# puzzlepaint/surfelmeshing

Hardware: AMD Instinct MI355X
Metric: RGB-D frames/s integrated @640x480, 5M live surfels; achieved HBM GB/s (higher is better)
Workload: dtype f32; 1 GPU; C2: synthetic room stream 640x480, raw depth + colour frames resident in HBM, full preprocessing + Integrate per frame, 4912850 live surfels (6250000 slots), steady-state re-traversal; max_surfel_count=6250000, streams=1, parallelism=1 independent stream per GPU

## Files before the change

include/smx.h:

```cpp
#ifndef SMX_H_
#define SMX_H_

#include <stddef.h>
#include <stdint.h>

#ifdef __cplusplus
extern "C" {
#endif

typedef enum {
  SMX_OK = 0,
  SMX_ERR_INVALID_ARGUMENT = -1,
  SMX_ERR_HIP = -2,
  SMX_ERR_NO_DEVICE = -3,
  SMX_ERR_UNSUPPORTED = -4
} smx_status;

typedef void* smx_stream;
typedef struct smx_buffer_s* smx_buffer;
typedef struct smx_recon_s* smx_recon;
typedef struct smx_nn_s* smx_nn;

typedef struct {
  void* address;
// ... 150 lines not shown
int smx_recon_debug_internal_stream(smx_recon r, smx_stream* out);
int smx_recon_debug_stamp_ring(smx_recon r, uint64_t* out, int32_t capacity_words, int32_t* wall_clock_khz);
int smx_recon_set_timing_enabled(smx_recon r, int32_t enabled);
int smx_recon_kernel_slot_count(void);
const char* smx_recon_kernel_slot_name(int32_t slot);
int smx_recon_get_kernel_timings(smx_recon r, float* out_ms, int32_t capacity);
int smx_recon_profile_begin(smx_recon r, int32_t slot, int32_t max_frames);
int smx_recon_profile_end(smx_recon r, float* avg_ms, int32_t* frames);
int smx_recon_counts(smx_recon r, smx_stream s, uint32_t* surfel_count, uint32_t* surfels_size);

typedef struct {
  uint32_t surfels_size, merge_count;
  uint32_t n_visible;
  uint32_t n_new, n_merged, n_recent, n_edges;
  uint32_t n_integrated, n_replaced, n_conflict_hits;
  uint32_t capacity_clamped;
  uint32_t n_window_edges;
  uint32_t n_contributors;
  uint32_t n_segments_skipped;
  uint32_t regularizer_saturated;
  uint32_t n_pairs;
  uint32_t n_overflow_pairs;
  uint32_t max_tile_pairs;
} smx_recon_stats;
int smx_recon_get_stats(smx_recon r, smx_stream s, smx_recon_stats* out);
int smx_recon_set_stats_enabled(smx_recon r, int32_t enabled);

int smx_recon_debug_download_surfels(smx_recon r, smx_stream s, float* rows, uint32_t count);
int smx_recon_debug_upload_surfels(smx_recon r, smx_stream s, const float* rows, uint32_t count,
                                   uint32_t merge_count);
enum {
  SMX_SCRATCH_SUPPORTING = 0,
  SMX_SCRATCH_SUPPORT_COUNTS = 1,
  SMX_SCRATCH_DEPTH_SUMS = 2,
  SMX_SCRATCH_CONFLICTING = 3,
  SMX_SCRATCH_FIRST_DEPTH = 4,
  SMX_SCRATCH_NEW_FLAGS = 5,
  SMX_SCRATCH_NEW_INDICES = 6
};
int smx_recon_debug_download_scratch(smx_recon r, smx_stream s, int32_t which, void* dst);
int smx_recon_debug_count_skipped_segments(smx_recon r, smx_stream s, uint32_t* out);
int smx_recon_set_scan_mode(smx_recon r, int32_t mode);
int smx_recon_debug_set_skip(smx_recon r, int32_t mask);
int smx_recon_set_overlap(smx_recon r, int32_t enabled);
int smx_recon_integrate_hooks(smx_recon r, smx_event inputs_consumed, smx_event chain_after);
int smx_recon_integrate_inputs_ready(smx_recon r, smx_event inputs_ready);
// ... 520 lines not shown
```

surfelmeshing_amd/_lib.py:

```python
import ctypes as C
import os

os.environ.setdefault("GPU_MAX_HW_QUEUES", "8")
_HERE = os.path.dirname(os.path.abspath(__file__))
SO_PATH = os.environ.get("SMX_LIB_PATH") or os.path.join(_HERE, "libsmx.so")


class SmxError(RuntimeError):
    pass


class BufferDesc(C.Structure):
    _fields_ = [("address", C.c_void_p), ("height", C.c_int32), ("width", C.c_int32), ("pitch", C.c_size_t)]


class IntegrateParams(C.Structure):
    _fields_ = [("sensor_noise_factor", C.c_float),
                ("max_surfel_confidence", C.c_float),
                ("regularizer_weight", C.c_float),
                ("regularization_frame_window_size", C.c_int32),
                ("do_blending", C.c_int32),
                ("measurement_blending_radius", C.c_int32),
                ("regularization_iterations_per_integration_iteration", C.c_int32),
                ("radius_factor_for_regularization_neighbors", C.c_float),
# ... 325 lines not shown
    _fields_ = [(n, C.c_uint32) for n in ("n_in", "n_out_of_range", "n_not_live", "n_clipped", "n_degenerate", "n_culled",
                                          "n_drawn", "n_large", "n_covered_pixels")]


class SurfelBuffersCPU(C.Structure):
    _fields_ = [("frame_index", C.c_uint32), ("surfel_count", C.c_size_t),
                ("surfel_x_buffer", C.c_void_p), ("surfel_y_buffer", C.c_void_p), ("surfel_z_buffer", C.c_void_p),
                ("surfel_radius_squared_buffer", C.c_void_p),
                ("surfel_normal_x_buffer", C.c_void_p), ("surfel_normal_y_buffer", C.c_void_p),
                ("surfel_normal_z_buffer", C.c_void_p), ("surfel_last_update_stamp_buffer", C.c_void_p)]


class SurfelDeltaCPU(C.Structure):
    _fields_ = [("capacity", C.c_uint32), ("count", C.c_uint32), ("frame_index", C.c_uint32), ("surfel_count", C.c_uint32),
                ("surfel_index", C.c_void_p), ("x", C.c_void_p), ("y", C.c_void_p), ("z", C.c_void_p),
                ("radius_squared", C.c_void_p), ("normal_x", C.c_void_p), ("normal_y", C.c_void_p),
                ("normal_z", C.c_void_p), ("last_update_stamp", C.c_void_p)]


class ReconStats(C.Structure):
    _fields_ = [(n, C.c_uint32) for n in
                ("surfels_size", "merge_count", "n_visible", "n_new", "n_merged", "n_recent", "n_edges",
                 "n_integrated", "n_replaced", "n_conflict_hits", "capacity_clamped", "n_window_edges", "n_contributors",
                 "n_segments_skipped", "regularizer_saturated", "n_pairs", "n_overflow_pairs", "max_tile_pairs")]


class NNStats(C.Structure):
    _fields_ = [("n_points", C.c_uint32), ("n_indexed", C.c_uint32), ("n_bricks", C.c_uint32), ("cell_size", C.c_float),
                ("dim", C.c_int32 * 3), ("key_bits", C.c_int32), ("tiles", C.c_uint64), ("staged_candidates", C.c_uint64),
                ("distance_tests", C.c_uint64), ("results", C.c_uint64)]


EXPORTS = [
    "smx_last_error", "smx_runtime_advice", "smx_host_is_page_locked", "smx_device_count", "smx_set_device", "smx_device_name",
    "smx_stream_create", "smx_stream_create_with_priority", "smx_stream_create_with_cu_mask", "smx_recon_set_internal_cu_mask", "smx_recon_set_handover_mode", "smx_recon_get_handover_mode", "smx_host_alloc", "smx_host_free", "smx_stream_destroy", "smx_stream_synchronize", "smx_debug_marker", "smx_debug_handover_probe",
    "smx_debug_live_allocations", "smx_debug_fail_allocation",
    "smx_event_create", "smx_event_create_timed", "smx_event_elapsed_ms", "smx_event_destroy", "smx_event_record", "smx_stream_wait_event",
    "smx_buffer_create", "smx_buffer_destroy", "smx_buffer_get_desc", "smx_buffer_upload", "smx_buffer_upload_by_kernel", "smx_buffer_download",
    "smx_buffer_upload_part", "smx_buffer_download_part", "smx_buffer_clear", "smx_buffer_set_to",
    "smx_bilateral_filtering_and_depth_cutoff", "smx_outlier_depth_map_fusion", "smx_bilateral_outlier_fusion", "smx_erode_depth_map",
    "smx_copy_without_border", "smx_median_filter_and_densify_depth_map", "smx_downscale_using_median_while_excluding", "smx_color_image_pyramid", "smx_compute_normals_and_drop_bad_pixels",
    "smx_compute_point_radii_and_remove_isolated_pixels", "smx_erode_normals_radii", "smx_erode_normals_radii_signal",
    "smx_recon_create", "smx_recon_destroy", "smx_recon_integrate", "smx_recon_regularize",
    "smx_recon_transfer_all_to_cpu", "smx_recon_set_delta_tracking", "smx_recon_transfer_changed_to_cpu", "smx_recon_export_vertices", "smx_recon_get_timings", "smx_recon_get_timings_nowait", "smx_recon_debug_stamp_ring", "smx_recon_debug_internal_stream",
    "smx_recon_build_neighbor_index", "smx_recon_neighbor_candidates", "smx_recon_check_triangles",
    "smx_mesh_params_default", "smx_recon_triangulate", "smx_recon_debug_mesh_timings",
    "smx_recon_triangulate_update", "smx_recon_triangulate_reset", "smx_recon_debug_mesh_update_timings", "smx_recon_deform_by_creation_frame",
# ... 62 lines not shown
```

surfelmeshing_amd/csrc/smx_recon.hip:

```cpp
#include <math.h>
#include <cmath>
#include <stdlib.h>
#include <string.h>

#include <algorithm>
#include <atomic>
#include <vector>

#include "smx_recon_state.hpp"
#include "smx_mesh.hpp"
#include <hip/hip_ext.h>

using namespace smx;

namespace {

struct FrameCtx {
  Mat34 L;
  Mat34 G;
  float fx, fy, cx, cy;
  Unproj up;
  float inv_depth_scaling;
  float sensor_noise_factor;
  float cos_normal_compat;
// ... 165 lines not shown

__device__ __forceinline__ void keep(uint32_t v) { asm volatile("" :: "v"(v)); }
__device__ __forceinline__ void keep(int v) { asm volatile("" :: "v"(v)); }
__device__ __forceinline__ void keep(float v) { asm volatile("" :: "v"(v)); }
__device__ __forceinline__ void keep(const float2& v) { keep(v.x); keep(v.y); }
__device__ __forceinline__ void keep(const float4& v) { keep(v.x); keep(v.y); keep(v.z); keep(v.w); }
__device__ __forceinline__ void keep(const uint2& v) { keep(v.x); keep(v.y); }
__device__ __forceinline__ void keep(const uint4& v) { keep(v.x); keep(v.y); keep(v.z); keep(v.w); }

__device__ __forceinline__ void SMX_SET_WAVE_PRIO() { __builtin_amdgcn_s_setprio(1); }
typedef uint32_t v4u_t __attribute__((ext_vector_type(4)));
__device__ __forceinline__ void out_store16(void* p, const v4u_t& w) { *reinterpret_cast<v4u_t*>(p) = w; }
__device__ __forceinline__ void out_store16(void* p, const uint4& v) { const v4u_t w = {v.x, v.y, v.z, v.w}; out_store16(p, w); }
__device__ __forceinline__ void out_store16(void* p, const float4& v) {
  const v4u_t w = {__float_as_uint(v.x), __float_as_uint(v.y), __float_as_uint(v.z), __float_as_uint(v.w)};
  out_store16(p, w);
}
__device__ __forceinline__ void out_store16(void* p, unsigned long long a, unsigned long long b) {
  const v4u_t w = {(uint32_t)a, (uint32_t)(a >> 32), (uint32_t)b, (uint32_t)(b >> 32)};
  out_store16(p, w);
}

__global__ void k_reset_frame_stats(DevState* st, int cull_only) {
  if (cull_only) { st->n_segments_skipped = 0; return; }
  st->n_visible = 0; st->n_merged = 0; st->n_integrated = 0; st->n_replaced = 0; st->n_conflict_hits = 0;
  st->n_pairs = 0; st->n_overflow_pairs = 0; st->max_tile_pairs = 0;
}

__global__ void __launch_bounds__(kBlock)
k_cull_segments(FrameCtx c, Lists L, SegWork sw, DevState* st, uint32_t nseg_alloc, uint32_t max_new_slots, unsigned long long ts_seq) {
  SMX_SET_WAVE_PRIO();
  if (c.ts && blockIdx.x == 0 && threadIdx.x == 0) {
#pragma unroll
    for (int k = 2; k < kTsWords; ++k) c.ts[k] = 0;
    c.ts[kTsSeq] = ts_seq;
    c.ts[kTsCullBegin] = wall_clock64();
  }
  const uint32_t seg = blockIdx.x * kBlock + threadIdx.x;
  const bool have_seg = seg < nseg_alloc;
  const uint32_t sidx = have_seg ? seg : 0u;
  const float4 b0 = *reinterpret_cast<const float4*>(&L.seg_box[8 * (size_t)sidx]);
  const float4 b1 = *reinterpret_cast<const float4*>(&L.seg_box[8 * (size_t)sidx + 4]);
  const uint32_t vis_prev = L.vis_seg[sidx];
  const uint32_t streak = L.seg_streak[sidx];
  const uint32_t n_bound = st->surfel_count + max_new_slots;
  const bool mine = have_seg && (unsigned long long)seg * kSeg < (unsigned long long)n_bound;
  bool skip = false;
  if (mine && __float_as_uint(b1.z) == (uint32_t)kSeg && vis_prev == 0 &&
      stamp_outside_window(__float_as_uint(b1.w), c.frame, c.reg_window)) {
    const Vec3 lo = {b0.x, b0.y, b0.z}, hi = {b0.w, b1.x, b1.y};
    skip = box_out_of_view(lo, hi, c);
  }
  const bool survive = mine && !skip, copy = skip && streak < 2u;
  if (skip) {
    L.seg_act[seg] = 0;
    if (streak < 255u) L.seg_streak[seg] = (uint8_t)(streak + 1u);
  } else if (mine && streak) {
    L.seg_streak[seg] = 0;
  }
  __shared__ uint32_t wave_n[2][kBlock / 64], list_base[2];
  const unsigned long long sm = __ballot(survive), cm = __ballot(copy);
  const uint32_t lane = threadIdx.x & 63u, wave = threadIdx.x >> 6;
  if (lane == 0) { wave_n[0][wave] = (uint32_t)__popcll(sm); wave_n[1][wave] = (uint32_t)__popcll(cm); }
  __syncthreads();
  if (threadIdx.x < 2) {
    uint32_t total = 0;
#pragma unroll
    for (int w = 0; w < kBlock / 64; ++w) total += wave_n[threadIdx.x][w];
    list_base[threadIdx.x] = total ? atomicAdd(&sw.count[threadIdx.x], total) : 0u;
  }
  __syncthreads();
  uint32_t sbase = list_base[0], cbase = list_base[1];
#pragma unroll
  for (int w = 0; w < kBlock / 64; ++w)
    if ((uint32_t)w < wave) { sbase += wave_n[0][w]; cbase += wave_n[1][w]; }
  const unsigned long long below = (1ull << lane) - 1ull;
  if (survive) sw.surv_list[sbase + (uint32_t)__popcll(sm & below)] = seg;
  if (copy) sw.copy_list[cbase + (uint32_t)__popcll(cm & below)] = seg;
  if (c.stats) {
    const unsigned long long km = __ballot(skip);
    if (lane == 0 && km) atomicAdd(&st->n_segments_skipped, (uint32_t)__popcll(km));
  }
}

__global__ void __launch_bounds__(kBlock, 8)
k_scan_visible(Surfels S, FrameCtx c, Lists L, TileBins tb, SegWork sw, const uint8_t* __restrict__ flags_prev, DevState* st,
               int use_lds_tables) {
  SMX_SET_WAVE_PRIO();
  ts_begin(c.ts, kTsScanBegin);
  __shared__ uint32_t wave_tot[kBlock / 64];
  __shared__ float box_part[kBlock / 64][8];
  __shared__ uint32_t pair_key[kPairHash], pair_cnt[kPairHash];
  __shared__ uint32_t vis_run_pos;
  const bool lds_tables = use_lds_tables != 0;
  const uint32_t G = gridDim.x, wg = blockIdx.x;
  const uint32_t n_surv = sw.count[0], n_copy = sw.count[1];
  uint32_t next_seg = sw.surv_list[wg];
  const uint32_t N = st->surfel_count;
  for (uint32_t e = wg; e < n_copy; e += G) {
    const uint32_t i0 = sw.copy_list[e] * (uint32_t)kSeg + threadIdx.x * 4;
    if (i0 < N) {
      const uchar4 of = *reinterpret_cast<const uchar4*>(&flags_prev[i0]);
      *reinterpret_cast<uchar4*>(&L.flags8[i0]) = make_uchar4(of.x & 2u, of.y & 2u, of.z & 2u, of.w & 2u);
    }
  }
  bool first_segment = true;
#pragma unroll 1
  for (uint32_t e = wg; e < n_surv; e += G) {
    {
      const uint32_t seg_id = next_seg;
      uint32_t tid = threadIdx.x;
      asm volatile("" : "+v"(tid));
      const uint32_t base = seg_id * (uint32_t)kSeg;
      const uint32_t i0 = base + tid * 4;
      const uint32_t il = i0 < N ? i0 : 0u;
      const float4* P = S.group(kGroupP, il);
      const float4 p0 = P[0], p1 = P[1], p2 = P[2], p3 = P[3];
      const uint32_t of_word = *reinterpret_cast<const uint32_t*>(&flags_prev[il]);
      next_seg = sw.surv_list[e + G < n_surv ? e + G : e];
      if (base >= N) continue;
      const uchar4 of = make_uchar4((uint8_t)(of_word & 255u), (uint8_t)((of_word >> 8) & 255u), (uint8_t)((of_word >> 16) & 255u), (uint8_t)(of_word >> 24));
      const uint32_t in_seg = (N - base < (uint32_t)kSeg) ? N - base : (uint32_t)kSeg;
      float* box = &L.seg_box[8 * (size_t)seg_id];
      if (!first_segment) __syncthreads();
      first_segment = false;
      if (lds_tables) {
#pragma unroll
        for (int k = 0; k < kPairHash / kBlock; ++k) { pair_key[k * kBlock + tid] = kInvalid; pair_cnt[k * kBlock + tid] = 0; }
        __syncthreads();
      }
      uint32_t vis_bits = 0;
      bool lane_recent = false;
      float bmin[3] = {3.0e38f, 3.0e38f, 3.0e38f}, bmax[3] = {-3.0e38f, -3.0e38f, -3.0e38f};
      uint32_t newest = 0;
      bool have_stamp = false;
      uint32_t key[8];
#pragma unroll
      for (int j = 0; j < 8; ++j) key[j] = kNoPair;
      if (i0 < N) {
        const uint32_t stamps[4] = {__float_as_uint(p0.w), __float_as_uint(p1.w), __float_as_uint(p2.w), __float_as_uint(p3.w)};
        const float xs[4] = {p0.x, p1.x, p2.x, p3.x};
        const float ys[4] = {p0.y, p1.y, p2.y, p3.y};
        const float zs[4] = {p0.z, p1.z, p2.z, p3.z};
        const uint8_t old_flags[4] = {of.x, of.y, of.z, of.w};
        uint8_t new_flags[4];
#pragma unroll
        for (int j = 0; j < 4; ++j) {
          const uint32_t i = i0 + j;
          new_flags[j] = (uint8_t)((old_flags[j] & 2u) | (stamp_outside_window(stamps[j], c.frame, c.reg_window) ? 0u : 1u));
          Proj p;
          const Vec3 g = {xs[j], ys[j], zs[j]};
          if (i < N) {
            bmin[0] = fminf(bmin[0], g.x); bmin[1] = fminf(bmin[1], g.y); bmin[2] = fminf(bmin[2], g.z);
            bmax[0] = fmaxf(bmax[0], g.x); bmax[1] = fmaxf(bmax[1], g.y); bmax[2] = fmaxf(bmax[2], g.z);
            if (!have_stamp || (int)stamps[j] > (int)newest) { newest = stamps[j]; have_stamp = true; }
          }
          if (i < N && maybe_in_image(g, c) && project_pos(g, c, p)) {
            vis_bits |= 1u << j;
            const bool active = is_active(stamps[j], c.frame, c.window);
            if (active && c.stats) atomicAdd(&st->n_visible, 1u);
            const uint32_t act = active ? kPairActive : 0u;
            key[2 * j] = (((uint32_t)(p.py / kTileH) * (uint32_t)tb.tiles_x + (uint32_t)(p.px / kTileW)) << 10) |
                         (uint32_t)((p.py % kTileH) * kTileW + (p.px % kTileW)) | act;
            int ox, oy;
            if (active && quadrant(p, c, ox, oy))
              key[2 * j + 1] = (((uint32_t)(oy / kTileH) * (uint32_t)tb.tiles_x + (uint32_t)(ox / kTileW)) << 10) |
                               (uint32_t)((oy % kTileH) * kTileW + (ox % kTileW)) | act | kPairSecond;
          }
        }
        *reinterpret_cast<uchar4*>(&L.flags8[i0]) = make_uchar4(new_flags[0], new_flags[1], new_flags[2], new_flags[3]);
        lane_recent = ((new_flags[0] | new_flags[1] | new_flags[2] | new_flags[3]) & 1u) != 0;
      }
      uint32_t rank[8];
#pragma unroll
      for (int j = 0; j < 8; ++j) {
        rank[j] = kInvalid;
        if (key[j] != kNoPair && lds_tables) {
          const uint32_t tile = key[j] >> 10;
          uint32_t h = (tile * 2654435761u) >> 16;
          for (int probe = 0; probe < 16; ++probe) {
            h &= (uint32_t)kPairHash - 1u;
            const uint32_t seen = atomicCAS(&pair_key[h], kInvalid, tile);
            if (seen == kInvalid || seen == tile) { rank[j] = (h << 16) | atomicAdd(&pair_cnt[h], 1u); break; }
            ++h;
          }
        }
      }
      const bool wave_recent = __ballot(lane_recent) != 0;
      if (wave_recent && (tid & 63) == 0) L.hot_epoch[base >> L.hot_shift] = (uint8_t)L.epoch;
      int newest_s = have_stamp ? (int)newest : (int)0x80000000;
#pragma unroll
      for (int off = 32; off > 0; off >>= 1) {
#pragma unroll
        for (int k = 0; k < 3; ++k) {
          bmin[k] = fminf(bmin[k], __shfl_xor(bmin[k], off));
          bmax[k] = fmaxf(bmax[k], __shfl_xor(bmax[k], off));
        }
        const int o = __shfl_xor(newest_s, off);
        newest_s = o > newest_s ? o : newest_s;
      }
      if ((tid & 63) == 0) {
        float* bp = box_part[tid >> 6];
        bp[0] = bmin[0]; bp[1] = bmin[1]; bp[2] = bmin[2]; bp[3] = bmax[0]; bp[4] = bmax[1]; bp[5] = bmax[2];
        bp[6] = __int_as_float(newest_s);
        bp[7] = wave_recent ? 1.0f : 0.0f;
      }
      uint32_t total;
      uint32_t off = block_excl_scan((uint32_t)__popc(vis_bits), wave_tot, total);
      uint32_t run_pos = 0;
      if (tid == 0 && total) run_pos = atomicAdd(&L.vis_chunks.count[(e % kSubLists) * kCountStride], total);
      if (lds_tables) {
// ... 18 lines not shown
      for (int j = 0; j < 4; ++j)
        if (vis_bits & (1u << j)) L.vis_list[off++] = i0 + j;
      if (lds_tables) {
#pragma unroll
        for (int j = 0; j < 8; ++j)
          if (key[j] != kNoPair)
            pair_store(tb, key[j], i0 + (uint32_t)(j >> 1),
                       rank[j] != kInvalid ? pair_key[rank[j] >> 16] + (rank[j] & 0xFFFFu) : atomicAdd(&tb.count[(key[j] >> 10) * kCountStride], 1u));
      } else {
#pragma unroll
        for (int j = 0; j < 8; ++j)
          if (key[j] != kNoPair) pair_store(tb, key[j], i0 + (uint32_t)(j >> 1), atomicAdd(&tb.count[(key[j] >> 10) * kCountStride], 1u));
      }
      if (tid == 0) {
        L.vis_seg[seg_id] = total;
        L.seg_act[seg_id] = (total != 0 || box_part[0][7] + box_part[1][7] + box_part[2][7] + box_part[3][7] != 0.0f) ? 1 : 0;
        float lo[3] = {3.0e38f, 3.0e38f, 3.0e38f}, hi[3] = {-3.0e38f, -3.0e38f, -3.0e38f};
        int ns = (int)0x80000000;
        for (int w = 0; w < kBlock / 64; ++w) {
          for (int k = 0; k < 3; ++k) { lo[k] = fminf(lo[k], box_part[w][k]); hi[k] = fmaxf(hi[k], box_part[w][3 + k]); }
          const int o = __float_as_int(box_part[w][6]);
          ns = o > ns ? o : ns;
        }
        box[0] = lo[0]; box[1] = lo[1]; box[2] = lo[2]; box[3] = hi[0]; box[4] = hi[1]; box[5] = hi[2];
        box[6] = __uint_as_float(in_seg);
        box[7] = __int_as_float(ns);
      }
    }
  }
}

template <bool kUseList>
__device__ __forceinline__ uint32_t walk_begin(const Chunks& ch, uint32_t n_slots_scan, uint32_t first, uint32_t& desc, uint32_t& cntv) {
  if (kUseList) {
    desc = ch.desc[(size_t)(first % kSubLists) * ch.stride + first / kSubLists];
    cntv = ch.count[(threadIdx.x % kSubLists) * kCountStride];
    keep(desc); keep(cntv);
    uint32_t longest = cntv;
#pragma unroll
    for (uint32_t off = kSubLists / 2; off > 0; off >>= 1) longest = max(longest, (uint32_t)__shfl_xor((int)longest, (int)off));
    return __builtin_amdgcn_readfirstlane(longest) * kSubLists;
  }
  desc = 0; cntv = 0;
  return (n_slots_scan + kBlock - 1) / kBlock;
}
template <bool kUseList>
// ... 1864 lines not shown

int read_surfel_count(smx_recon r, hipStream_t st, uint32_t* n) {
  SMX_HIP(hipMemcpyAsync(n, &r->st->surfel_count, sizeof(*n), hipMemcpyDeviceToHost, st));
  SMX_HIP(hipStreamSynchronize(st));
  return SMX_OK;
}

void enqueue_segment_scan(hipStream_t st, uint32_t* seg_count, int nseg, uint32_t* total_out) {
  hipLaunchKernelGGL(k_delta_scan, dim3(1), dim3(1024), 0, st, seg_count, nseg, total_out);
}

int acquire_staging(smx_recon r, hipStream_t st, size_t floats) {
  DevBuf<float>& buf = r->staging.buf;
  SMX_CALL(r->staging.mark.wait(st));
  if (buf.capacity() >= floats) return SMX_OK;
  if (buf.get()) SMX_HIP(hipDeviceSynchronize());
  return buf.alloc(floats, false);
}
int release_staging(smx_recon r, hipStream_t st) { return r->staging.mark.record(st); }

int invalidate_derived(smx_recon r, hipStream_t st) {
  SMX_HIP(hipMemsetAsync(r->L.vis_seg, 0, (size_t)r->nseg * 4, st));
  SMX_HIP(hipMemsetAsync(r->L.seg_box, 0, (size_t)r->nseg * 8 * sizeof(float), st));
  SMX_HIP(hipMemsetAsync(r->L.recent_seg, 0, (size_t)r->nsegB * 4, st));
  SMX_HIP(hipMemsetAsync(r->vis_count_set[0], 0, sizeof(uint32_t) * kSubLists * kCountStride, st));
  SMX_HIP(hipMemsetAsync(r->vis_count_set[1], 0, sizeof(uint32_t) * kSubLists * kCountStride, st));
  SMX_HIP(hipMemsetAsync(r->L.rec_chunks.count, 0, sizeof(uint32_t) * kSubLists * kCountStride, st));
  hipLaunchKernelGGL(k_rebuild_flags, dim3(r->grid_surfels), dim3(kBlock), 0, st, r->S, 0u, 0x7FFFFFFF, r->L.flags8, r->st);
  SMX_LAUNCH_CHECK();
  r->table_valid = false;
  r->hot_holdoff = 3;
  r->have_frame = false;
  return SMX_OK;
}

}

extern "C" {

int smx_recon_create(uint32_t max_surfel_count, int32_t width, int32_t height,
                     float fx, float fy, float cx, float cy, int32_t device_id, smx_recon* out) {
  SMX_CHECK_ARG(out != nullptr && max_surfel_count > 0 && max_surfel_count <= (1u << 30));
  SMX_CHECK_ARG(width >= 3 && height >= 3);
  int device = 0;
  SMX_CALL(resolve_device(device_id, &device));
  SMX_ON_DEVICE(device);
// ... 6 lines not shown
    }
  }
  smx_recon_s* r = new smx_recon_s();
  r->device = device;
  r->max_surfels = max_surfel_count;
  r->W = width; r->H = height; r->fx = fx; r->fy = fy; r->cx = cx; r->cy = cy;
  r->S.pitch = ((size_t)max_surfel_count + 63) / 64 * 64;
  const size_t P = (size_t)width * height;
  int rc;
#define SMX_TRY(x) do { rc = (x); if (rc != SMX_OK) { (void)smx_recon_destroy(r); return rc; } } while (0)
  SMX_TRY(r->mem.alloc(&r->S.base, (size_t)kQuadsPerSlot * 4 * r->S.pitch, true));
  SMX_TRY(r->mem.alloc(&r->grad_acc, 2 * ((size_t)r->S.pitch + kSegAcc), true));
  SMX_TRY(r->mem.alloc(&r->reg_rec, 2 * ((size_t)r->S.pitch + kSegAcc), true));
  r->nseg = div_up((long long)r->S.pitch, kSeg);
  r->nsegB = div_up((long long)r->S.pitch, kSegB);
  r->fb.cap = kFarBinCap; r->fb.hash_mask = (uint32_t)kFarHash - 1u;
  SMX_TRY(r->mem.alloc(&r->fb.rec, (size_t)r->nsegB * kFarBinCap, false));
  SMX_TRY(r->mem.alloc(&r->fb.count, ((size_t)r->nsegB + 1) * kCountStride, true));
  r->L.vis_region = (uint32_t)(div_up(r->nseg, kSubLists) * kSeg);
  SMX_TRY(r->mem.alloc(&r->L.vis_list, (size_t)kSubLists * r->L.vis_region, true));
  SMX_TRY(r->mem.alloc(&r->L.recent_list, (size_t)r->nsegB * kSegB, false));
  SMX_TRY(r->mem.alloc(&r->L.vis_seg, (size_t)r->nseg, true));
  SMX_TRY(r->mem.alloc(&r->L.seg_box, (size_t)r->nseg * 8, true));
  SMX_TRY(r->mem.alloc(&r->L.seg_act, (size_t)r->nseg, true));
  SMX_TRY(r->mem.alloc(&r->L.seg_streak, (size_t)r->nseg, true));
  SMX_TRY(r->mem.alloc(&r->sw.surv_list, (size_t)r->nseg + 65536, true));
  SMX_TRY(r->mem.alloc(&r->sw.copy_list, (size_t)r->nseg + 65536, true));
  SMX_TRY(r->mem.alloc(&r->sw.count, 2, true));
  SMX_TRY(r->mem.alloc_host(&r->dir_host, 2, true));
  r->dir_host[0] = 0;
  r->dir_host[1] = 0;
  SMX_TRY(hip_rc(hipHostGetDevicePointer(reinterpret_cast<void**>(&r->dir_dev), r->dir_host, 0), "hipHostGetDevicePointer"));
  SMX_TRY(r->mem.alloc(&r->L.recent_seg, (size_t)r->nsegB, true));
  r->L.vis_chunks.stride = 0; r->L.vis_chunks.desc = nullptr;
  r->L.rec_chunks.stride = (uint32_t)(div_up(r->nsegB, kSubLists) + 8192);
  SMX_TRY(r->mem.alloc(&r->L.rec_chunks.desc, (size_t)kSubLists * r->L.rec_chunks.stride, true));
  SMX_TRY(r->mem.alloc(&r->L.rec_chunks.count, (size_t)kSubLists * kCountStride, true));
  static_assert(kSegAcc == kSegB && kAccCount < kCountStride, "pass B lists the edge kernel's segments by its own segment numbers");
  r->L.acc_chunks.stride = r->L.rec_chunks.stride;
  r->L.acc_chunks.count = r->L.rec_chunks.count + kAccCount;
  SMX_TRY(r->mem.alloc(&r->L.acc_chunks.desc, (size_t)kSubLists * r->L.acc_chunks.stride, true));
  SMX_TRY(r->mem.alloc(&r->flags_buf[0], (size_t)r->nsegB * kSegB, true));
  SMX_TRY(r->mem.alloc(&r->flags_buf[1], (size_t)r->nsegB * kSegB, true));
  r->L.flags8 = r->flags_buf[0];
  r->L.hot_shift = 10;
  while ((((size_t)r->nseg * kSeg) >> r->L.hot_shift) + 1 > (size_t)kMaxHotGroups) ++r->L.hot_shift;
  r->L.n_hot_groups = (uint32_t)((((size_t)r->nseg * kSeg) >> r->L.hot_shift) + 1);
  SMX_TRY(r->mem.alloc(&r->L.hot_epoch, (size_t)r->L.n_hot_groups + 64, true));
  SMX_TRY(r->mem.alloc(&r->L.seg_targets, (size_t)r->nsegB * kBlockB, true));
  r->L.epoch = 128;
  r->L.plain_gathers = r->S.pitch >= kRangedGatherMaxPitch ? 1u : 0u;
  r->hot_filter_enabled = 1;
  r->fuse_edges = kFuseEdgesDefault;
  r->hot_holdoff = 3;
  SMX_TRY(r->mem.alloc(&r->merge_flag, r->S.pitch, true));
  SMX_TRY(r->mem.alloc(&r->gate_count, 32, true));
  r->gate_expected = 0;
  constexpr int kHandoverModeDefault = 1;
  r->handover_mode = kHandoverModeDefault;
  {
    const char* cc = getenv("ROCPROF_COUNTER_COLLECTION");
    if (cc && cc[0] && strcmp(cc, "0") != 0) r->handover_mode = 0;
  }
  SMX_TRY(r->mem.alloc(&r->L.act_list, (size_t)r->nsegB * kSegB, true));
  SMX_TRY(r->mem.alloc(&r->sc.supporting, P, true));
  SMX_TRY(r->mem.alloc(&r->sc.counts, P, true));
  SMX_TRY(r->mem.alloc(&r->sc.depth_sums, P, true));
  SMX_TRY(r->mem.alloc(&r->sc.assoc, P, true));
  for (int k = 0; k < 2; ++k) {
    SMX_TRY(r->mem.alloc(&r->vis_count_set[k], (size_t)kSubLists * kCountStride, true));
    SMX_TRY(r->mem.alloc(&r->ovf_count_set[k], 1, true));
  }
  r->L.vis_chunks.count = r->vis_count_set[0];
  r->tb.tiles_x = div_up(width, kTileW);
  r->tb.n_tiles = (uint32_t)(r->tb.tiles_x * div_up(height, kTileH));
// ... 126 lines not shown
}

int smx_recon_set_overlap(smx_recon r, int32_t enabled) {
  SMX_CHECK_ARG(r != nullptr && (enabled == 0 || enabled == 1));
  SMX_ON_DEVICE(r->device);
  if (r->reg_pending) { SMX_HIP(hipStreamSynchronize(r->reg_stream)); r->reg_pending = false; }
  r->overlap_enabled = enabled;
  return SMX_OK;
}

int smx_recon_set_handover_mode(smx_recon r, int32_t mode) {
  SMX_CHECK_ARG(r != nullptr && (mode == 0 || mode == 1));
  r->handover_mode = mode;
  return SMX_OK;
}

int smx_recon_get_handover_mode(smx_recon r, int32_t* mode) {
  SMX_CHECK_ARG(r != nullptr && mode != nullptr);
  *mode = r->handover_mode;
  return SMX_OK;
}

int smx_recon_set_scan_mode(smx_recon r, int32_t mode) {
  SMX_CHECK_ARG(r != nullptr && mode >= 0 && mode <= 2047);
  SMX_ON_DEVICE(r->device);
  r->grid_list = ((mode >> 8) & 1) ? 4 : r->grid_list_full;
  r->scan_mode = mode & 1;
  r->blend_multi_launch = (mode >> 1) & 1;
  r->hot_filter_enabled = ((mode >> 2) & 1) ? 0 : 1;
  r->tb.cap = ((mode >> 3) & 1) ? 16u : r->bin_cap_full;
  r->no_lds_tables = (mode >> 4) & 1;
  r->fb.cap = ((mode >> 5) & 1) ? 4u : kFarBinCap;
  r->fb.hash_mask = ((mode >> 6) & 1) ? 1u : (uint32_t)kFarHash - 1u;
  r->fuse_edges = ((mode >> 9) & 1) ? 1 : kFuseEdgesDefault;
  r->blend_other_tile = (mode >> 7) & 1;
  r->L.plain_gathers = (((mode >> 10) & 1) || r->S.pitch >= kRangedGatherMaxPitch) ? 1u : 0u;
  return SMX_OK;
}

int smx_recon_debug_set_skip(smx_recon r, int32_t mask) {
  SMX_CHECK_ARG(r != nullptr && mask >= 0 && mask <= 511);
  r->debug_skip = mask;
  return SMX_OK;
}

int smx_recon_integrate(smx_recon r, smx_stream s, uint32_t frame_index, float depth_scaling,
                        const smx_buffer_desc* depth, const smx_buffer_desc* normals,
                        const smx_buffer_desc* radius, const smx_buffer_desc* color,
                        const float global_T_local[12], const smx_integrate_params* p) {
  SMX_CHECK_ARG(r != nullptr);
  const hipEvent_t hook_consumed = r->hook_consumed, hook_chain = r->hook_chain, hook_ready = r->hook_ready;
  r->hook_consumed = nullptr; r->hook_chain = nullptr; r->hook_ready = nullptr;
  SMX_CHECK_ARG(depth && normals && radius && color && global_T_local && p);
  SMX_ON_DEVICE(r->device);
  SMX_CHECK_ARG(depth->width == r->W && depth->height == r->H && normals->width == r->W && normals->height == r->H);
  SMX_CHECK_ARG(radius->width == r->W && radius->height == r->H && color->width == r->W && color->height == r->H);
  SMX_CHECK_ARG(!p->do_blending || (p->measurement_blending_radius >= 2 && p->measurement_blending_radius <= 255));
  hipStream_t st = (hipStream_t)s;
  if (r->have_frame && (int32_t)(frame_index - r->last_frame) < 0) {
    SMX_CALL(join_regularizer(r, st));
    SMX_HIP(hipMemsetAsync(r->L.vis_seg, 0, (size_t)r->nseg * 4, st));
    SMX_HIP(hipMemsetAsync(r->L.seg_box, 0, (size_t)r->nseg * 8 * sizeof(float), st));
    r->hot_holdoff = 3;
  }
  r->have_frame = true; r->last_frame = frame_index;
  if (r->handover_mode == 1 && reinterpret_cast<volatile uint32_t*>(r->dir_host)[1] != 0u) r->handover_mode = 0;
  FrameCtx c;
  memcpy(c.G.m, global_T_local, sizeof(float) * 12);
  c.L = se3_inverse(global_T_local);
  c.fx = r->fx; c.fy = r->fy; c.cx = r->cx; c.cy = r->cy;
  c.up = make_unproj(r->fx, r->fy, r->cx, r->cy);
  c.inv_depth_scaling = 1.0f / depth_scaling;
  c.sensor_noise_factor = p->sensor_noise_factor;
  c.cos_normal_compat = cosf((float)(M_PI / 180.0f * p->normal_compatibility_threshold_deg));
  c.rf2 = p->radius_factor_for_regularization_neighbors * p->radius_factor_for_regularization_neighbors;
  c.max_conf = p->max_surfel_confidence;
  c.window = p->surfel_integration_active_window_size;
  c.reg_window = p->regularization_frame_window_size;
  c.frame = frame_index;
  c.W = r->W; c.H = r->H;
  c.stats = r->stats_enabled;
  c.ts = nullptr;
  if (r->timing_enabled & 4) { ++r->ts_seq; c.ts = r->ts_ring + (size_t)(r->ts_seq % kTsRing) * kTsWords; }
  const int P = r->W * r->H;
  const dim3 b(kBlock), gpx(div_up(P, kBlock)), gimg(div_up(r->W, 64), div_up(r->H, 4));
  const dim3 gs(r->nseg), gl(r->grid_list);
  const bool tm = (r->timing_enabled & 1) != 0;
  FrameIn in;
// ... 2 lines not shown
  const Img<uint16_t> depth_rw = as_img<uint16_t>(depth);

  const uint8_t* flags_prev = r->L.flags8;
  r->L.flags8 = (r->L.flags8 == r->flags_buf[0]) ? r->flags_buf[1] : r->flags_buf[0];
  r->L.epoch = (r->L.epoch + 1u) & 255u;
  if (r->hot_holdoff > 0) --r->hot_holdoff;
  const bool pipelined = r->overlap_enabled != 0;
  const hipStream_t sF = st;
  const hipStream_t sR = pipelined ? r->reg_stream : st;
  const bool split = pipelined && (r->debug_skip & 16) != 0;
  if (r->reg_pending && r->last_stream != st) SMX_CALL(join_regularizer(r, st));
  r->last_stream = st;
  if (r->stats_enabled) hipLaunchKernelGGL(k_reset_frame_stats, dim3(1), dim3(1), 0, sF, r->st, 1);
  if (tm) SMX_HIP(hipEventRecord(r->ev[0], sF));
  r->L.descending = *reinterpret_cast<volatile uint32_t*>(r->dir_host);
  r->sc_cur ^= 1;
  r->L.vis_chunks.count = r->vis_count_set[r->sc_cur];
  r->tb.ovf_count = r->ovf_count_set[r->sc_cur];
  if (hook_ready) SMX_HIP(hipStreamWaitEvent(sF, hook_ready, 0));
  {
    SlotTimer t(r, sF, kSlotCull);
    if (r->sw_dirty) SMX_HIP(hipMemsetAsync(r->sw.count, 0, 2 * sizeof(uint32_t), sF));
    r->sw_dirty = true;
    hipLaunchKernelGGL(k_cull_segments, dim3((unsigned)div_up(r->nseg, kBlock)), b, 0, sF, c, r->L, r->sw, r->st, (uint32_t)r->nseg, (uint32_t)P, r->ts_seq); }
  if (r->pending_mark) { SMX_HIP(hipStreamWaitEvent(sF, r->pending_mark, 0)); r->pending_mark = nullptr; }
  if (r->stats_enabled) hipLaunchKernelGGL(k_reset_frame_stats, dim3(1), dim3(1), 0, sF, r->st, 0);
  { SlotTimer t(r, sF, kSlotScanVisible, true);
    const bool lds_tables = !r->no_lds_tables;
    constexpr int kPassAWgsPerCu = 8;
    const dim3 ga((unsigned)(r->cu_count * kPassAWgsPerCu));
    hipExtLaunchKernelGGL(k_scan_visible, ga, b, 0, sF, t.start(), t.stop(), 0, r->S, c, r->L, r->tb, r->sw, flags_prev, r->st, lds_tables ? 1 : 0);
    r->table_valid = true; r->table_frame = frame_index; r->table_window = c.reg_window; }
  { SlotTimer t(r, sF, kSlotAssocTiles, true);
    hipExtLaunchKernelGGL(k_assoc_tiles, dim3(r->tb.n_tiles), dim3(kTilePx), 0, sF, t.start(), t.stop(), 0, r->S, c, r->sc, in.depth, in.normals, r->tb,
                       r->ovf_count_set[r->sc_cur ^ 1], r->merge_flag, r->st, r->L.seg_act, (uint32_t)r->nseg, r->dir_dev, r->sw.count,
                       r->stamps ? r->stamps : nullptr, r->ts_ring, c.ts ? r->ts_mapped_dev : nullptr, r->ts_seq);
    r->sw_dirty = false; }
  if (tm) { SMX_HIP(hipEventRecord(r->ev[1], sF)); SMX_HIP(hipEventRecord(r->ev[2], sF)); SMX_HIP(hipEventRecord(r->ev[3], sF)); SMX_HIP(hipEventRecord(r->ev[4], sF)); }
  const int halo = p->measurement_blending_radius - 1;
  const bool fused_blend = p->do_blending && halo <= kBlendMaxHalo && !r->blend_multi_launch;
  bool front_by_launch = false, front_by_gate = false;
  const float ds = 1.0f / c.inv_depth_scaling;
  const float term = p->do_blending ? 1.0f / ((float)p->measurement_blending_radius - 1.0f) : 0.0f;
  const Img<uint16_t> blended = {r->blended_depth, r->H, r->W, (size_t)r->W * sizeof(uint16_t)};
  if (fused_blend) {
    front_by_gate = pipelined && !split && r->handover_mode == 1 && !(r->debug_skip & 4) && !tm && !(r->timing_enabled & 2);
    SlotTimer t(r, sF, kSlotBlend, front_by_gate);
// ... 181 lines not shown
  SMX_CALL(check_handover(r, (hipStream_t)s));
  if (surfel_count) *surfel_count = h.surfel_count - h.merge_count;
  if (surfels_size) *surfels_size = h.surfel_count;
  return SMX_OK;
}

int smx_recon_get_stats(smx_recon r, smx_stream s, smx_recon_stats* out) {
  SMX_CHECK_ARG(r != nullptr && out != nullptr);
  SMX_ON_DEVICE(r->device);
  SMX_CALL(join_regularizer(r, (hipStream_t)s));
  DevState h;
  SMX_HIP(hipMemcpyAsync(&h, r->st, sizeof(h), hipMemcpyDeviceToHost, (hipStream_t)s));
  SMX_HIP(hipStreamSynchronize((hipStream_t)s));
  SMX_CALL(check_handover(r, (hipStream_t)s));
  out->surfels_size = h.surfel_count; out->merge_count = h.merge_count;
  out->n_visible = h.n_visible; out->n_new = h.new_count; out->n_merged = h.n_merged;
  out->n_recent = h.recent_count; out->n_edges = h.n_edges;
  out->n_integrated = h.n_integrated; out->n_replaced = h.n_replaced; out->n_conflict_hits = h.n_conflict_hits;
  out->capacity_clamped = h.capacity_clamped;
  out->n_window_edges = h.n_window_edges; out->n_contributors = h.n_contributors;
  out->n_segments_skipped = h.n_segments_skipped;
  out->regularizer_saturated = h.reg_saturated;
  out->n_pairs = h.n_pairs; out->n_overflow_pairs = h.n_overflow_pairs; out->max_tile_pairs = h.max_tile_pairs;
  return SMX_OK;
}

namespace {
bool stage_ms_from_stamps(const unsigned long long* t, unsigned long long seq, int khz, float out_ms[7]) {
  if (t[kTsSeq] != seq || t[kTsCullBegin] == 0) return false;
  auto ms = [&](unsigned long long a, unsigned long long b) { return (b > a && a != 0) ? (float)((double)(b - a) / (double)khz) : 0.0f; };
  auto first = [](unsigned long long a, unsigned long long b, unsigned long long c) { return a ? a : (b ? b : c); };
  const unsigned long long tiles_end = first(t[kTsBlendBegin], t[kTsTilesEnd], t[kTsCullBegin]);
  const unsigned long long int_end = first(t[kTsUpdBegin], t[kTsIntEnd], first(t[kTsIntBegin], t[kTsBlendEnd], tiles_end));
  const unsigned long long upd_end = first(t[kTsRegBegin], t[kTsUpdEnd], int_end);
  out_ms[0] = ms(t[kTsCullBegin], tiles_end);
  out_ms[1] = 0.0f;
  out_ms[2] = ms(tiles_end, t[kTsBlendEnd]);
  out_ms[3] = ms(t[kTsIntBegin], int_end);
  out_ms[4] = ms(int_end, upd_end);
  out_ms[5] = 0.0f;
  out_ms[6] = ms(upd_end, t[kTsRegEnd]);
  return true;
}
int copy_stamp_ring(smx_recon r) {
  SMX_HIP(hipMemcpy(r->ts_host, r->ts_ring, sizeof(unsigned long long) * kTsRing * kTsWords, hipMemcpyDeviceToHost));
  return SMX_OK;
// ... 147 lines not shown
```

surfelmeshing_amd/csrc/smx_recon_state.hpp:

```cpp
#pragma once

#include "smx_common.hpp"
#include "smx_components.hpp"
#include "smx_decimate.hpp"
#include "smx_distance.hpp"
#include "smx_fill.hpp"
#include "smx_raycast.hpp"
#include "smx_render.hpp"
#include "smx_rim.hpp"
#include "smx_sample.hpp"
#include "smx_track.hpp"

namespace smx {

struct MeshWorkspace;

enum : int {
  kX = 0, kY = 1, kZ = 2, kSmoothX = 3, kSmoothY = 4, kSmoothZ = 5, kConfidence = 6, kRadiusSq = 7,
  kNormalX = 8, kNormalY = 9, kNormalZ = 10, kGradX = 11, kGradY = 12, kGradZ = 13,
  kCreationStamp = 17, kLastUpdateStamp = 18, kNeighbor0 = 19, kGradCount = 23, kColor = 24, kRows = 25
};

struct DevState {
  uint32_t surfel_count;
  uint32_t merge_count;
  uint32_t create_base_next;
  uint32_t recent_count;
  uint32_t create_base;
  uint32_t new_count;
  uint32_t capacity_clamped;
  uint32_t n_visible, n_merged, n_edges, n_integrated, n_replaced, n_conflict_hits;
  uint32_t n_window_edges, n_contributors;
  uint32_t n_segments_skipped;
  uint32_t reg_saturated;
  uint32_t n_pairs, n_overflow_pairs, max_tile_pairs;
};

enum : int { kGroupP = 0, kGroupS, kGroupN, kGroupT, kGroupC, kGroupG, kGroups };
__host__ __device__ constexpr int row_group(int row) {
  return row <= 2 ? kGroupP : row <= 5 ? kGroupS : row == 6 ? kGroupC : row == 7 ? kGroupN : row <= 10 ? kGroupN
       : row <= 13 ? kGroupG : row <= 16 ? -1 : row == 17 ? kGroupC : row == 18 ? kGroupP : row <= 22 ? kGroupT
       : row == 24 ? kGroupC : -1;
}
__host__ __device__ constexpr int row_sub(int row) {
  return row <= 2 ? row : row <= 5 ? row - 3 : row == 6 ? 0 : row == 7 ? 3 : row <= 10 ? row - 8
       : row <= 13 ? row - 11 : row == 17 ? 1 : row == 18 ? 3 : row <= 22 ? row - 19 : row == 24 ? 2 : -1;
}
__host__ __device__ constexpr int group_start(int g) { return g; }
constexpr int kQuadsPerSlot = 6;
struct Surfels {
  float* base;
  size_t pitch;
  __host__ __device__ __forceinline__ size_t quad(int g, uint32_t i) const { return (size_t)group_start(g) * pitch + (size_t)i; }
  __device__ __forceinline__ float& f(int row, uint32_t i) const { return base[quad(row_group(row), i) * 4 + row_sub(row)]; }
  __device__ __forceinline__ uint32_t& u(int row, uint32_t i) const {
    return reinterpret_cast<uint32_t*>(base)[quad(row_group(row), i) * 4 + row_sub(row)];
  }
  __device__ __forceinline__ float4* group(int g, uint32_t i) const { return reinterpret_cast<float4*>(base) + quad(g, i); }
// ... 13 lines not shown
constexpr int kBlock = 256;

inline unsigned blocks_for(uint32_t n) { return (unsigned)div_up(n, kBlock); }
inline bool finite_f(float v) { return v - v == 0.0f; }
inline bool ranges_overlap(const void* a, size_t a_bytes, const void* b, size_t b_bytes) {
  if (!a || !b || a_bytes == 0 || b_bytes == 0) return false;
  const uintptr_t a0 = (uintptr_t)a, b0 = (uintptr_t)b;
  return a0 < b0 + b_bytes && b0 < a0 + a_bytes;
}
inline unsigned long long word64(const uint32_t* h, int lo) { return ((unsigned long long)h[lo + 1] << 32) | h[lo]; }

constexpr int kSeg = 1024;
constexpr int kSegB = 1024;
constexpr int kBlockB = kSegB / 4;
constexpr uint32_t kCountStride = 32;
constexpr uint32_t kSubLists = 16;
struct Chunks { uint32_t* desc; uint32_t* count; uint32_t stride; };
struct Lists {
  Chunks vis_chunks, rec_chunks;
  Chunks acc_chunks;
  uint32_t* vis_list;
  uint32_t vis_region;
  float* seg_box;
  uint32_t* vis_seg;
  uint8_t* seg_streak;
  uint32_t* recent_list;
  uint32_t* recent_seg;
  uint32_t* act_list;
  uint8_t* flags8;
  uint8_t* dirty8;
  uint8_t* seg_act;
  uint32_t descending;
  uint32_t plain_gathers;
  uint8_t* hot_epoch;
  uint16_t* seg_targets;
  uint32_t n_hot_groups;
  uint32_t epoch;
  int hot_shift;
};

struct FarBins {
  uint4* rec;
  uint32_t* count;
  uint32_t cap;
  uint32_t hash_mask;
};
// ... 125 lines not shown
  uint32_t table_frame;
  int table_window;
  int stats_enabled;
  hipEvent_t hook_consumed, hook_chain;
  hipEvent_t hook_ready;
  int blend_multi_launch;
  smx::Scratch sc;
  smx::TileBins tb;
  smx::SegWork sw;
  bool sw_dirty;
  hipEvent_t pending_mark;
  uint32_t* ovf_count_set[2];
  unsigned long long* stamps;
  int no_lds_tables;
  int blend_other_tile;
  int cu_count;
  uint32_t bin_cap_full;
  uint32_t* vis_count_set[2];
  uint32_t* dir_host;
  uint32_t* dir_dev;
  int sc_cur;
  int hot_holdoff;
  int hot_filter_enabled;
  int fuse_edges;
  uint16_t* blended_depth;
  smx::BlendBufs bb;
  uint8_t* new_flags;
  uint32_t* new_ranks;
  uint32_t* block_sums;
  uint32_t* block_offsets;
  uint32_t* tmp_u32;
  int n_scan_blocks;
  smx::DevState* st;
  int scan_mode;
  int timing_enabled;
  bool have_timings;
  unsigned long long* ts_ring;
  unsigned long long* ts_host;
  volatile unsigned long long* ts_mapped;
  unsigned long long* ts_mapped_dev;
  unsigned long long ts_seq;
  int wall_khz;
  hipEvent_t ev[14];
  hipEvent_t kev[2 * 16];
  bool kev_recorded[16];
  int prof_slot;
  int prof_cap, prof_n;
  hipEvent_t* prof_ev;
  smx::DevBuf<uint8_t> dirty;
  smx::DevBuf<uint32_t> delta_seg;
  smx::DevBuf<uint32_t> delta_total;
  int grid_surfels;
  int grid_list;
  int grid_acc;
  int grid_list_full;
  int debug_skip;
  int overlap_enabled;
  hipStream_t reg_stream;
  uint32_t* gate_count;
  uint32_t gate_expected;
  int handover_mode;
  hipEvent_t ev_front;
  hipEvent_t ev_upd;
  hipEvent_t ev_reg;
  bool reg_pending;
  hipStream_t last_stream;
  uint8_t* flags_buf[2];
  bool have_frame;
  uint32_t last_frame;
  smx::StagingWork staging;
  smx::RenderWork render;
  smx::TrackWork track;
  smx::DecimateWork decimate;
  smx::ComponentsWork components;
  smx::FillWork fill;
  smx::DistanceWork distance;
  smx::RimWork rim;
  smx::RaycastWork raycast;
  smx::SampleWork sample;
  smx::CompareWork compare;
  smx::RegisterMeshWork register_mesh;
  smx::CompactWork compact;
  smx::CandidateWork candidates;
  smx::MeshWorkspace* mesh;
};

namespace smx {

int join_regularizer(smx_recon r, hipStream_t st);
int read_surfel_count(smx_recon r, hipStream_t st, uint32_t* n);
void enqueue_segment_scan(hipStream_t st, uint32_t* seg_count, int nseg, uint32_t* total_out);
int acquire_staging(smx_recon r, hipStream_t st, size_t floats);
// ... 5 lines not shown
```

Before: 6190 frames/s.

## Park out-of-view segments whose recent stamps cannot intersect the regularization window

Adds a per-segment 64-bit mask of recent update stamps (mod 64), built during the visibility scan. The cull kernel uses it to 'park' segments that are out of view and whose in-window stamps cannot matter for the current frame's table span, even when the newest stamp is still inside the window. Parked segments skip the full per-surfel scan and only copy or mark their flags, keeping bits 0 and 1. This cuts re-traversal bandwidth for the steady-state scan, at the cost of an extra 8-byte-per-segment array, more streak bookkeeping, and correctness that depends on the table-window conditions.

```diff
diff --git a/include/smx.h b/include/smx.h
--- a/include/smx.h
+++ b/include/smx.h
@@ -196,6 +196,7 @@
   uint32_t n_pairs;
   uint32_t n_overflow_pairs;
   uint32_t max_tile_pairs;
+  uint32_t n_segments_parked;
 } smx_recon_stats;
 int smx_recon_get_stats(smx_recon r, smx_stream s, smx_recon_stats* out);
 int smx_recon_set_stats_enabled(smx_recon r, int32_t enabled);
diff --git a/surfelmeshing_amd/_lib.py b/surfelmeshing_amd/_lib.py
--- a/surfelmeshing_amd/_lib.py
+++ b/surfelmeshing_amd/_lib.py
@@ -371,7 +371,8 @@
     _fields_ = [(n, C.c_uint32) for n in
                 ("surfels_size", "merge_count", "n_visible", "n_new", "n_merged", "n_recent", "n_edges",
                  "n_integrated", "n_replaced", "n_conflict_hits", "capacity_clamped", "n_window_edges", "n_contributors",
-                 "n_segments_skipped", "regularizer_saturated", "n_pairs", "n_overflow_pairs", "max_tile_pairs")]
+                 "n_segments_skipped", "regularizer_saturated", "n_pairs", "n_overflow_pairs", "max_tile_pairs",
+                 "n_segments_parked")]
 
 
 class NNStats(C.Structure):
diff --git a/surfelmeshing_amd/csrc/smx_recon.hip b/surfelmeshing_amd/csrc/smx_recon.hip
--- a/surfelmeshing_amd/csrc/smx_recon.hip
+++ b/surfelmeshing_amd/csrc/smx_recon.hip
@@ -211,13 +211,15 @@
 }
 
 __global__ void k_reset_frame_stats(DevState* st, int cull_only) {
-  if (cull_only) { st->n_segments_skipped = 0; return; }
+  if (cull_only) { st->n_segments_skipped = 0; st->n_segments_parked = 0; return; }
   st->n_visible = 0; st->n_merged = 0; st->n_integrated = 0; st->n_replaced = 0; st->n_conflict_hits = 0;
   st->n_pairs = 0; st->n_overflow_pairs = 0; st->max_tile_pairs = 0;
 }
 
+constexpr uint32_t kCopyKeep = 0x80000000u, kCopyMarkOnly = 0x40000000u, kCopySegMask = 0x3FFFFFFFu;
 __global__ void __launch_bounds__(kBlock)
-k_cull_segments(FrameCtx c, Lists L, SegWork sw, DevState* st, uint32_t nseg_alloc, uint32_t max_new_slots, unsigned long long ts_seq) {
+k_cull_segments(FrameCtx c, Lists L, SegWork sw, DevState* st, uint32_t nseg_alloc, uint32_t max_new_slots, unsigned long long ts_seq,
+                int park_on, unsigned long long park_test) {
   SMX_SET_WAVE_PRIO();
   if (c.ts && blockIdx.x == 0 && threadIdx.x == 0) {
 #pragma unroll
@@ -231,24 +233,33 @@
   const float4 b0 = *reinterpret_cast<const float4*>(&L.seg_box[8 * (size_t)sidx]);
   const float4 b1 = *reinterpret_cast<const float4*>(&L.seg_box[8 * (size_t)sidx + 4]);
   const uint32_t vis_prev = L.vis_seg[sidx];
-  const uint32_t streak = L.seg_streak[sidx];
+  const uint32_t streak_byte = L.seg_streak[sidx];
+  const unsigned long long stamp_mask = L.seg_mask[sidx];
   const uint32_t n_bound = st->surfel_count + max_new_slots;
   const bool mine = have_seg && (unsigned long long)seg * kSeg < (unsigned long long)n_bound;
-  bool skip = false;
-  if (mine && __float_as_uint(b1.z) == (uint32_t)kSeg && vis_prev == 0 &&
-      stamp_outside_window(__float_as_uint(b1.w), c.frame, c.reg_window)) {
-    const Vec3 lo = {b0.x, b0.y, b0.z}, hi = {b0.w, b1.x, b1.y};
-    skip = box_out_of_view(lo, hi, c);
-  }
-  const bool survive = mine && !skip, copy = skip && streak < 2u;
-  if (skip) {
-    L.seg_act[seg] = 0;
-    if (streak < 255u) L.seg_streak[seg] = (uint8_t)(streak + 1u);
-  } else if (mine && streak) {
+  bool skip = false, park = false;
+  if (mine && __float_as_uint(b1.z) == (uint32_t)kSeg && vis_prev == 0) {
+    const bool cold = stamp_outside_window(__float_as_uint(b1.w), c.frame, c.reg_window);
+    if (cold || (park_on && (stamp_mask & park_test) == 0ull)) {
+      const Vec3 lo = {b0.x, b0.y, b0.z}, hi = {b0.w, b1.x, b1.y};
+      const bool out = box_out_of_view(lo, hi, c);
+      skip = out && cold;
+      park = out && !cold;
+    }
+  }
+  const uint32_t streak = ((streak_byte >> 7) == (park ? 1u : 0u)) ? (streak_byte & 127u) : 0u;
+  const bool survive = mine && !skip && !park, copy = skip && streak < 2u;
+  if (skip || park) {
+    if (skip) L.seg_act[seg] = 0;
+    const uint32_t next = (streak < 127u ? streak + 1u : 127u) | (park ? 128u : 0u);
+    if (next != streak_byte) L.seg_streak[seg] = (uint8_t)next;
+  } else if (mine && streak_byte) {
     L.seg_streak[seg] = 0;
   }
+  const bool listed = copy || park;
+  const uint32_t list_entry = seg | (park ? kCopyKeep | (streak < 2u ? 0u : kCopyMarkOnly) : 0u);
   __shared__ uint32_t wave_n[2][kBlock / 64], list_base[2];
-  const unsigned long long sm = __ballot(survive), cm = __ballot(copy);
+  const unsigned long long sm = __ballot(survive), cm = __ballot(listed);
   const uint32_t lane = threadIdx.x & 63u, wave = threadIdx.x >> 6;
   if (lane == 0) { wave_n[0][wave] = (uint32_t)__popcll(sm); wave_n[1][wave] = (uint32_t)__popcll(cm); }
   __syncthreads();
@@ -265,10 +276,11 @@
     if ((uint32_t)w < wave) { sbase += wave_n[0][w]; cbase += wave_n[1][w]; }
   const unsigned long long below = (1ull << lane) - 1ull;
   if (survive) sw.surv_list[sbase + (uint32_t)__popcll(sm & below)] = seg;
-  if (copy) sw.copy_list[cbase + (uint32_t)__popcll(cm & below)] = seg;
+  if (listed) sw.copy_list[cbase + (uint32_t)__popcll(cm & below)] = list_entry;
   if (c.stats) {
-    const unsigned long long km = __ballot(skip);
+    const unsigned long long km = __ballot(skip), pm = __ballot(park);
     if (lane == 0 && km) atomicAdd(&st->n_segments_skipped, (uint32_t)__popcll(km));
+    if (lane == 0 && pm) atomicAdd(&st->n_segments_parked, (uint32_t)__popcll(pm));
   }
 }
 
@@ -279,6 +291,7 @@
   ts_begin(c.ts, kTsScanBegin);
   __shared__ uint32_t wave_tot[kBlock / 64];
   __shared__ float box_part[kBlock / 64][8];
+  __shared__ unsigned long long mask_part[kBlock / 64];
   __shared__ uint32_t pair_key[kPairHash], pair_cnt[kPairHash];
   __shared__ uint32_t vis_run_pos;
   const bool lds_tables = use_lds_tables != 0;
@@ -287,10 +300,14 @@
   uint32_t next_seg = sw.surv_list[wg];
   const uint32_t N = st->surfel_count;
   for (uint32_t e = wg; e < n_copy; e += G) {
-    const uint32_t i0 = sw.copy_list[e] * (uint32_t)kSeg + threadIdx.x * 4;
-    if (i0 < N) {
+    const uint32_t entry = sw.copy_list[e];
+    const uint32_t seg_base = (entry & kCopySegMask) * (uint32_t)kSeg;
+    const uint32_t i0 = seg_base + threadIdx.x * 4;
+    const uint32_t keep_bits = (entry & kCopyKeep) ? 3u : 2u;
+    if ((entry & kCopyKeep) && threadIdx.x == 0) L.hot_epoch[seg_base >> L.hot_shift] = (uint8_t)L.epoch;
+    if (i0 < N && !(entry & kCopyMarkOnly)) {
       const uchar4 of = *reinterpret_cast<const uchar4*>(&flags_prev[i0]);
-      *reinterpret_cast<uchar4*>(&L.flags8[i0]) = make_uchar4(of.x & 2u, of.y & 2u, of.z & 2u, of.w & 2u);
+      *reinterpret_cast<uchar4*>(&L.flags8[i0]) = make_uchar4(of.x & keep_bits, of.y & keep_bits, of.z & keep_bits, of.w & keep_bits);
     }
   }
   bool first_segment = true;
@@ -323,6 +340,23 @@
       float bmin[3] = {3.0e38f, 3.0e38f, 3.0e38f}, bmax[3] = {-3.0e38f, -3.0e38f, -3.0e38f};
       uint32_t newest = 0;
       bool have_stamp = false;
+      {
+        unsigned long long stamp_mask = 0;
+        const uint32_t st4[4] = {__float_as_uint(p0.w), __float_as_uint(p1.w), __float_as_uint(p2.w), __float_as_uint(p3.w)};
+        uint32_t i0m = i0;
+        asm volatile("" : "+v"(i0m));
+#pragma unroll
+        for (int j = 0; j < 4; ++j) {
+          uint32_t sj = st4[j];
+          asm volatile("" : "+v"(sj));
+          if (i0m + j < N && !stamp_outside_window(sj, c.frame, c.reg_window)) stamp_mask |= 1ull << (sj & 63u);
+        }
+        if (__ballot(stamp_mask != 0ull) != 0ull) {
+#pragma unroll
+          for (int off = 32; off > 0; off >>= 1) stamp_mask |= __shfl_xor(stamp_mask, off);
+        }
+        if ((tid & 63) == 0) mask_part[tid >> 6] = stamp_mask;
+      }
       uint32_t key[8];
 #pragma unroll
       for (int j = 0; j < 8; ++j) key[j] = kNoPair;
@@ -360,6 +394,7 @@
         *reinterpret_cast<uchar4*>(&L.flags8[i0]) = make_uchar4(new_flags[0], new_flags[1], new_flags[2], new_flags[3]);
         lane_recent = ((new_flags[0] | new_flags[1] | new_flags[2] | new_flags[3]) & 1u) != 0;
       }
+      const bool wave_recent = __ballot(lane_recent) != 0;
       uint32_t rank[8];
 #pragma unroll
       for (int j = 0; j < 8; ++j) {
@@ -375,7 +410,6 @@
           }
         }
       }
-      const bool wave_recent = __ballot(lane_recent) != 0;
       if (wave_recent && (tid & 63) == 0) L.hot_epoch[base >> L.hot_shift] = (uint8_t)L.epoch;
       int newest_s = have_stamp ? (int)newest : (int)0x80000000;
 #pragma unroll
@@ -440,6 +474,7 @@
           const int o = __float_as_int(box_part[w][6]);
           ns = o > ns ? o : ns;
         }
+        L.seg_mask[seg_id] = mask_part[0] | mask_part[1] | mask_part[2] | mask_part[3];
         box[0] = lo[0]; box[1] = lo[1]; box[2] = lo[2]; box[3] = hi[0]; box[4] = hi[1]; box[5] = hi[2];
         box[6] = __uint_as_float(in_seg);
         box[7] = __int_as_float(ns);
@@ -2350,6 +2385,7 @@
 int invalidate_derived(smx_recon r, hipStream_t st) {
   SMX_HIP(hipMemsetAsync(r->L.vis_seg, 0, (size_t)r->nseg * 4, st));
   SMX_HIP(hipMemsetAsync(r->L.seg_box, 0, (size_t)r->nseg * 8 * sizeof(float), st));
+  SMX_HIP(hipMemsetAsync(r->L.seg_mask, 0, (size_t)r->nseg * sizeof(unsigned long long), st));
   SMX_HIP(hipMemsetAsync(r->L.recent_seg, 0, (size_t)r->nsegB * 4, st));
   SMX_HIP(hipMemsetAsync(r->vis_count_set[0], 0, sizeof(uint32_t) * kSubLists * kCountStride, st));
   SMX_HIP(hipMemsetAsync(r->vis_count_set[1], 0, sizeof(uint32_t) * kSubLists * kCountStride, st));
@@ -2402,6 +2438,7 @@
   SMX_TRY(r->mem.alloc(&r->L.recent_list, (size_t)r->nsegB * kSegB, false));
   SMX_TRY(r->mem.alloc(&r->L.vis_seg, (size_t)r->nseg, true));
   SMX_TRY(r->mem.alloc(&r->L.seg_box, (size_t)r->nseg * 8, true));
+  SMX_TRY(r->mem.alloc(&r->L.seg_mask, (size_t)r->nseg, true));
   SMX_TRY(r->mem.alloc(&r->L.seg_act, (size_t)r->nseg, true));
   SMX_TRY(r->mem.alloc(&r->L.seg_streak, (size_t)r->nseg, true));
   SMX_TRY(r->mem.alloc(&r->sw.surv_list, (size_t)r->nseg + 65536, true));
@@ -2431,6 +2468,7 @@
   r->L.epoch = 128;
   r->L.plain_gathers = r->S.pitch >= kRangedGatherMaxPitch ? 1u : 0u;
   r->hot_filter_enabled = 1;
+  r->park_enabled = 1;
   r->fuse_edges = kFuseEdgesDefault;
   r->hot_holdoff = 3;
   SMX_TRY(r->mem.alloc(&r->merge_flag, r->S.pitch, true));
@@ -2603,7 +2641,7 @@
 }
 
 int smx_recon_set_scan_mode(smx_recon r, int32_t mode) {
-  SMX_CHECK_ARG(r != nullptr && mode >= 0 && mode <= 2047);
+  SMX_CHECK_ARG(r != nullptr && mode >= 0 && mode <= 4095);
   SMX_ON_DEVICE(r->device);
   r->grid_list = ((mode >> 8) & 1) ? 4 : r->grid_list_full;
   r->scan_mode = mode & 1;
@@ -2615,6 +2653,7 @@
   r->fb.hash_mask = ((mode >> 6) & 1) ? 1u : (uint32_t)kFarHash - 1u;
   r->fuse_edges = ((mode >> 9) & 1) ? 1 : kFuseEdgesDefault;
   r->blend_other_tile = (mode >> 7) & 1;
+  r->park_enabled = ((mode >> 11) & 1) ? 0 : 1;
   r->L.plain_gathers = (((mode >> 10) & 1) || r->S.pitch >= kRangedGatherMaxPitch) ? 1u : 0u;
   return SMX_OK;
 }
@@ -2642,9 +2681,23 @@
     SMX_CALL(join_regularizer(r, st));
     SMX_HIP(hipMemsetAsync(r->L.vis_seg, 0, (size_t)r->nseg * 4, st));
     SMX_HIP(hipMemsetAsync(r->L.seg_box, 0, (size_t)r->nseg * 8 * sizeof(float), st));
+    SMX_HIP(hipMemsetAsync(r->L.seg_mask, 0, (size_t)r->nseg * sizeof(unsigned long long), st));
     r->hot_holdoff = 3;
   }
-  r->have_frame = true; r->last_frame = frame_index;
+  int park_on = 0;
+  unsigned long long park_test = 0;
+  {
+    const int w = p->regularization_frame_window_size;
+    const uint32_t span = frame_index - r->table_frame;
+    if (r->park_enabled && r->have_frame && r->table_valid && r->table_window == w && r->last_reg_window == w && w >= 0 && w <= 62 &&
+        span < 64u - (uint32_t)w && (int32_t)(frame_index - (uint32_t)w) >= (int32_t)(r->table_frame - (uint32_t)w)) {
+      park_on = 1;
+      const unsigned long long run = (1ull << span) - 1ull;
+      const uint32_t first = (r->table_frame - (uint32_t)w) & 63u;
+      park_test = first ? (run << first) | (run >> (64u - first)) : run;
+    }
+  }
+  r->have_frame = true; r->last_frame = frame_index; r->last_reg_window = p->regularization_frame_window_size;
   if (r->handover_mode == 1 && reinterpret_cast<volatile uint32_t*>(r->dir_host)[1] != 0u) r->handover_mode = 0;
   FrameCtx c;
   memcpy(c.G.m, global_T_local, sizeof(float) * 12);
@@ -2693,7 +2746,8 @@
     SlotTimer t(r, sF, kSlotCull);
     if (r->sw_dirty) SMX_HIP(hipMemsetAsync(r->sw.count, 0, 2 * sizeof(uint32_t), sF));
     r->sw_dirty = true;
-    hipLaunchKernelGGL(k_cull_segments, dim3((unsigned)div_up(r->nseg, kBlock)), b, 0, sF, c, r->L, r->sw, r->st, (uint32_t)r->nseg, (uint32_t)P, r->ts_seq); }
+    hipLaunchKernelGGL(k_cull_segments, dim3((unsigned)div_up(r->nseg, kBlock)), b, 0, sF, c, r->L, r->sw, r->st, (uint32_t)r->nseg, (uint32_t)P, r->ts_seq,
+                       park_on, park_test); }
   if (r->pending_mark) { SMX_HIP(hipStreamWaitEvent(sF, r->pending_mark, 0)); r->pending_mark = nullptr; }
   if (r->stats_enabled) hipLaunchKernelGGL(k_reset_frame_stats, dim3(1), dim3(1), 0, sF, r->st, 0);
   { SlotTimer t(r, sF, kSlotScanVisible, true);
@@ -2921,6 +2975,7 @@
   out->n_segments_skipped = h.n_segments_skipped;
   out->regularizer_saturated = h.reg_saturated;
   out->n_pairs = h.n_pairs; out->n_overflow_pairs = h.n_overflow_pairs; out->max_tile_pairs = h.max_tile_pairs;
+  out->n_segments_parked = h.n_segments_parked;
   return SMX_OK;
 }
 
diff --git a/surfelmeshing_amd/csrc/smx_recon_state.hpp b/surfelmeshing_amd/csrc/smx_recon_state.hpp
--- a/surfelmeshing_amd/csrc/smx_recon_state.hpp
+++ b/surfelmeshing_amd/csrc/smx_recon_state.hpp
@@ -34,6 +34,7 @@
   uint32_t n_segments_skipped;
   uint32_t reg_saturated;
   uint32_t n_pairs, n_overflow_pairs, max_tile_pairs;
+  uint32_t n_segments_parked;
 };
 
 enum : int { kGroupP = 0, kGroupS, kGroupN, kGroupT, kGroupC, kGroupG, kGroups };
@@ -93,6 +94,7 @@
   uint32_t* vis_list;
   uint32_t vis_region;
   float* seg_box;
+  unsigned long long* seg_mask;
   uint32_t* vis_seg;
   uint8_t* seg_streak;
   uint32_t* recent_list;
@@ -264,6 +266,7 @@
   int sc_cur;
   int hot_holdoff;
   int hot_filter_enabled;
+  int park_enabled;
   int fuse_edges;
   uint16_t* blended_depth;
   smx::BlendBufs bb;
@@ -310,6 +313,7 @@
   uint8_t* flags_buf[2];
   bool have_frame;
   uint32_t last_frame;
+  int last_reg_window;
   smx::StagingWork staging;
   smx::RenderWork render;
   smx::TrackWork track;
```

After: 6161 frames/s. No clear change (-0.5%).
